# g8a9/multi-modal-emotion

Hardware: AMD Instinct MI355X
Metric: utterances/sec fwd+bwd (+clip_grad_norm_+AdamW inside the timed step), TAV (BERT+Wav2Vec2+VideoMAE) b=32, 1/2/4/8 MI355X (higher is better)
Workload: dtype bf16; 1 GPU; tav_nn.py TAV preset B (bert 12 L + wav2vec2 12 L / 768 + videomae 12 L / 768 on 16 frames + fusion 12 L), global batch 32 = 32 per GPU x 1, text 128 tok, audio 80000 samples, video 16x3x224x224 (104 fusion / 1464 encoder tokens), 547.0 GFLOP forward per utterance; global_batch=32, per_gpu_batch=32, parallelism=dp1, weights=random init (seeded), no checkpoints offline, launch=hipGraph replay

## Files before the change

### multi-modal-emotion_amd/csrc/attention.hip

```cpp
#include "common.h"
#include <type_traits>
#include "tavhip_internal.h"


namespace tav {

struct AttnP {
    const char* q; const char* k; const char* v; char* o; char* o_soft;
    const float* mask; float* lse; float* corr;
    const char* dout; char* dq; char* dk; char* dv; float* delta;
    int B, S, nh;
    long ld_q, ld_k, ld_v, ld_o, ld_do, ld_dq, ld_dk, ld_dv;
    float scale;
    int pre;
    int tiles;
};
struct AttnPL : AttnP { const int* lens; };
template <bool LEN> using AttnArg = std::conditional_t<LEN, AttnPL, AttnP>;

struct AttnTile { int x, head, b; };
TAV_DEV AttnTile attn_tile(const AttnP& p) {
    const int id = xcd_remap((int)blockIdx.x, (int)gridDim.x);
    const int hb = id / p.tiles, b = hb / p.nh;
    AttnTile w;
// ... 26 lines not shown
    static constexpr int NSD = ROWCH / 4;
    static constexpr int PITCH_N = ROWB + (ES == 2 ? 32 : 16);
    static constexpr bool DUAL = (ES == 2);
    static TAV_DEV int row_off(int row, int chunk) {
        return row * ROWB + ((chunk ^ (ES == 2 ? (((row >> 1) & 3) << 1) : (row & 15))) << 4);
    }
};

TAV_DEV uint4 frag_tr_rowimg(const char* img, int krow0, int dt, int lane) {
    using H = HD<bf16>;
    const int g = lane >> 4, i = lane & 15, q = i >> 2, p = i & 3;
    const int r0 = krow0 + 4 * g + q, r1 = r0 + 16;
    const uint2 lo = lds_read_tr16(img + H::row_off(r0, 2 * dt + (p >> 1)) + 8 * (p & 1));
    const uint2 hi = lds_read_tr16(img + H::row_off(r1, 2 * dt + (p >> 1)) + 8 * (p & 1));
    return make_uint4(lo.x, lo.y, hi.x, hi.y);
}
template <typename T> TAV_DEV float tile_elem(const char* rowimg, const char* natimg, int row, int d) {
    if constexpr (HD<T>::DUAL) return ET<T>::ld(reinterpret_cast<const T*>(rowimg + HD<T>::row_off(row, d >> 3)) + (d & 7));
    else return ET<T>::ld(reinterpret_cast<const T*>(natimg + row * HD<T>::PITCH_N) + d);
}
template <typename T> TAV_DEV uint4 tile_kfrag(const char* rowimg, const char* natimg, int krow0, int dt, int lane) {
    if constexpr (HD<T>::DUAL) return frag_tr_rowimg(rowimg, krow0, dt, lane);
    else return frag_kstrided<T>(natimg, HD<T>::PITCH_N, krow0, 16 * dt, lane);
}

template <typename T, int ROWS, int N>
TAV_DEV void tile_addr_init(unsigned (&off0)[N], unsigned (&offmax)[N], long ld_bytes, int S, int tid) {
    constexpr int ROWCH = HD<T>::ROWCH;
    static_assert(N == ROWS * ROWCH / 256, "chunks per thread");
#pragma unroll
    for (int e = 0; e < N; ++e) {
        const int idx = tid + 256 * e, row = idx / ROWCH, ch = idx - row * ROWCH;
        off0[e] = (unsigned)(row * ld_bytes + ch * 16);
        offmax[e] = (unsigned)((S - 1) * ld_bytes + ch * 16);
    }
}
template <int N>
TAV_DEV void tile_gload(uint4 (&regs)[N], const char* base, const unsigned (&off0)[N], const unsigned (&offmax)[N], unsigned tile_off) {
#pragma unroll
    for (int e = 0; e < N; ++e) {
        unsigned o = off0[e] + tile_off;
        o = o < offmax[e] ? o : offmax[e];
        typedef unsigned u32x4 __attribute__((ext_vector_type(4)));
        const u32x4 v = *reinterpret_cast<const u32x4*>(base + o);
        regs[e] = make_uint4(v.x, v.y, v.z, v.w);
    }
}

template <typename T, int ROWS>
TAV_DEV void tile_zero_pad(uint4* regs, int row0, int S, int tid) {
    constexpr int ROWCH = HD<T>::ROWCH, N = ROWS * ROWCH / 256;
#pragma unroll
    for (int e = 0; e < N; ++e) {
        const int idx = tid + 256 * e, row = idx / ROWCH;
        if (row0 + row >= S) regs[e] = make_uint4(0, 0, 0, 0);
    }
}
template <typename T, int ROWS>
TAV_DEV void tile_lstore_row(const uint4* regs, char* img, int tid) {
    constexpr int ROWCH = HD<T>::ROWCH, N = ROWS * ROWCH / 256;
#pragma unroll
    for (int e = 0; e < N; ++e) {
        const int idx = tid + 256 * e, row = idx / ROWCH, ch = idx - row * ROWCH;
        *reinterpret_cast<uint4*>(img + HD<T>::row_off(row, ch)) = regs[e];
    }
}
template <typename T, int ROWS>
TAV_DEV void tile_lstore_nat(const uint4* regs, char* img, int tid) {
    constexpr int ROWCH = HD<T>::ROWCH, N = ROWS * ROWCH / 256;
#pragma unroll
    for (int e = 0; e < N; ++e) {
        const int idx = tid + 256 * e, row = idx / ROWCH, ch = idx - row * ROWCH;
        *reinterpret_cast<uint4*>(img + row * HD<T>::PITCH_N + ch * 16) = regs[e];
    }
}

template <typename T>
TAV_DEV void row_frags_gload(uint4* f, const char* base, long ld_bytes, int r, int S, int g) {
    if (r >= S) r = S - 1;
#pragma unroll
    for (int s = 0; s < HD<T>::NSD; ++s) f[s] = *reinterpret_cast<const uint4*>(base + (long)r * ld_bytes + (4 * s + g) * 16);
}

template <int ROWS = 64> struct PairDmaT {
    static constexpr int NP = ROWS / 32;
    const char* a; const char* b;
    unsigned lda_b, ldb_b;
    unsigned offa[NP], offb[NP];
    unsigned lds_a, lds_b;
    int S, wave;
    TAV_DEV void init(const char* a_, const char* b_, long lda_bytes, long ldb_bytes, int S_, const void* lds_img_a, const void* lds_img_b, int tid) {
        a = a_; b = b_; lda_b = (unsigned)lda_bytes; ldb_b = (unsigned)ldb_bytes; S = S_;
        const int lane = tid & 63;
        wave = tid >> 6;
#pragma unroll
        for (int j = 0; j < NP; ++j) {
            const int row = wave * 8 * NP + j * 8 + (lane >> 3), slot = lane & 7;
            const int ch = slot ^ (((row >> 1) & 3) << 1);
            offa[j] = (unsigned)row * lda_b + (unsigned)(ch * 16);
            offb[j] = (unsigned)row * ldb_b + (unsigned)(ch * 16);
        }
        lds_a = __builtin_amdgcn_readfirstlane(lds_addr(lds_img_a) + wave * 8 * NP * 128);
        lds_b = __builtin_amdgcn_readfirstlane(lds_addr(lds_img_b) + wave * 8 * NP * 128);
    }
    template <bool RAGGED> TAV_DEV void issue(int t, unsigned slot_bytes) const {
        const char* ab = a + (size_t)t * (unsigned)ROWS * lda_b;
        const char* bb = b + (size_t)t * (unsigned)ROWS * ldb_b;
        unsigned oa[NP], ob[NP];
#pragma unroll
        for (int j = 0; j < NP; ++j) { oa[j] = offa[j]; ob[j] = offb[j]; }
        if constexpr (RAGGED) {
            int ln = threadIdx.x & 63;
            asm volatile("" : "+v"(ln));
#pragma unroll
            for (int j = 0; j < NP; ++j) {
                const int over = t * ROWS + wave * 8 * NP + j * 8 + (ln >> 3) - (S - 1);
                if (over > 0) { oa[j] -= (unsigned)over * lda_b; ob[j] -= (unsigned)over * ldb_b; }
            }
        }
        if constexpr (NP == 2) glds16_x4(ab, bb, oa[0], oa[1], ob[0], ob[1], lds_a + slot_bytes, lds_b + slot_bytes);
        else glds16_x2(ab, bb, oa[0], ob[0], lds_a + slot_bytes, lds_b + slot_bytes);
    }
};
using PairDma = PairDmaT<64>;

constexpr int ATT_FWD_OCC = 3;
constexpr float ATT_LAZY_THR = 12.0f;
constexpr int ATT_FWD_NQ = 2;
template <typename T, int MODE, bool PRE, bool LEN = false>
__global__ __launch_bounds__(256, ATT_FWD_OCC) void attn_fwd_kernel(const AttnArg<LEN> p) {
    constexpr int NQ = ATT_FWD_NQ;
    using H = HD<T>;
    constexpr int ES = H::ES, NSD = H::NSD, KSTEP = ET<T>::KSTEP, BKV = 64;
    constexpr int NCH = BKV * H::ROWCH / 256;
    constexpr bool DMA = ES == 2;
    constexpr int KROW_B = BKV * H::ROWB, VNAT_B = DMA ? BKV * H::ROWB : BKV * H::PITCH_N;
    constexpr int BUF_B = KROW_B + VNAT_B + 2 * BKV * 4;
    constexpr int NBUF = 2;
    extern __shared__ __attribute__((aligned(16))) char smem[];
    float* red = reinterpret_cast<float*>(smem + NBUF * BUF_B);

    const int tid = threadIdx.x, lane = tid & 63, wave = tid >> 6, g = lane >> 4, i = lane & 15;
    const AttnTile wg = attn_tile(p);
    const int head = wg.head, b = wg.b, S = p.S, L = valid_len<LEN>(p, b);
    const int q0 = wg.x * (64 * NQ) + wave * (16 * NQ);
    if constexpr (LEN) {
        if (wg.x * (64 * NQ) >= L) {
            zero_head_rows<T>(p.o, p.ld_o, b, S, head, wg.x * (64 * NQ), 64 * NQ, tid);
            if (MODE == 2) zero_head_rows<T>(p.o_soft, p.ld_o, b, S, head, wg.x * (64 * NQ), 64 * NQ, tid);
            if (tid < 64 * NQ && wg.x * (64 * NQ) + tid < S) p.lse[((long)b * p.nh + head) * S + wg.x * (64 * NQ) + tid] = 0.f;
            if (MODE == 2 && wg.x == 0 && tid < 64) p.corr[((long)b * p.nh + head) * 64 + tid] = 0.f;
            return;
        }
    }
    const long hoff = (long)head * 64 * ES;
    const char* Qb = p.q + (long)b * S * p.ld_q * ES + hoff;
    const char* Kb = p.k + (long)b * S * p.ld_k * ES + hoff;
    const char* Vb = p.v + (long)b * S * p.ld_v * ES + hoff;
    const float* maskb = p.mask ? p.mask + (long)b * S : nullptr;

    uint4 qf[NQ][NSD];
#pragma unroll
    for (int qt = 0; qt < NQ; ++qt) row_frags_gload<T>(qf[qt], Qb, p.ld_q * ES, q0 + 16 * qt + i, L, g);

    constexpr float LOG2E = 1.4426950408889634f;
    const float c2 = PRE ? 1.0f : p.scale * LOG2E;
    const uint4 ones = (ES == 2) ? make_uint4(0x3F803F80u, 0x3F803F80u, 0x3F803F80u, 0x3F803F80u)
                                 : make_uint4(0x3F800000u, 0x3F800000u, 0x3F800000u, 0x3F800000u);
    uint4 ones_v = ones;
    asm volatile("" : "+v"(ones_v.x), "+v"(ones_v.y), "+v"(ones_v.z), "+v"(ones_v.w));
    unsigned koff[NSD], vtoff[4];
    if constexpr (ES == 2) {
#pragma unroll
        for (int s = 0; s < NSD; ++s) { koff[s] = (unsigned)H::row_off(i, 4 * s + g); asm volatile("" : "+v"(koff[s])); }
#pragma unroll
        for (int dt = 0; dt < 4; ++dt) {
            vtoff[dt] = (unsigned)(H::row_off(4 * g + (i >> 2), 2 * dt + ((i & 3) >> 1)) + 8 * (i & 1));
            asm volatile("" : "+v"(vtoff[dt]));
        }
    }
    float m_run[NQ];
    f32x4 mneg[NQ];
    f32x4 lacc[NQ];
    f32x4 oacc[4][NQ];
#pragma unroll
    for (int qt = 0; qt < NQ; ++qt) {
        m_run[qt] = -1e30f;
        mneg[qt] = f32x4{0.f, 0.f, 0.f, 0.f};
        lacc[qt] = f32x4{0.f, 0.f, 0.f, 0.f};
#pragma unroll
        for (int a = 0; a < 4; ++a) oacc[a][qt] = f32x4{0.f, 0.f, 0.f, 0.f};
    }
    float corr_part = 0.f;
// ... 183 lines not shown
                f32x4 tl[2];
                tl[0] = sacc[ks * ET<T>::ACC_TILES][qt];
                tl[1] = sacc[ks * ET<T>::ACC_TILES + ET<T>::ACC_TILES - 1][qt];
                pb[qt] = acc_to_kfrag<T>(tl);
            }
#pragma unroll
            for (int qt = 0; qt < NQ; ++qt) mma16<T>(ones_v, pb[qt], lacc[qt]);
#pragma unroll
            for (int dt = 0; dt < 4; ++dt) {
                uint4 a;
                if constexpr (DMA) {
                    const char* vt = Vnat + vtoff[dt] + ks * KSTEP * H::ROWB;
                    const uint2 lo = lds_read_tr16(vt), hi = lds_read_tr16(vt + 16 * H::ROWB);
                    a = make_uint4(lo.x, lo.y, hi.x, hi.y);
                }
                else a = frag_kstrided<T>(Vnat, H::PITCH_N, ks * KSTEP, 16 * dt, lane);
#pragma unroll
                for (int qt = 0; qt < NQ; ++qt) mma16<T>(a, pb[qt], oacc[dt][qt]);
            }
        }
        if (MODE == 2) {
            const int d = tid & 63, kq = tid >> 6;
#pragma unroll 4
            for (int kk = 0; kk < 16; ++kk) {
                const int key = kq * 16 + kk;
                if constexpr (DMA) corr_part += cm[key] * ET<T>::ld(reinterpret_cast<const T*>(Vnat + H::row_off(key, d >> 3)) + (d & 7));
                else corr_part += cm[key] * ET<T>::ld(reinterpret_cast<const T*>(Vnat + key * H::PITCH_N) + d);
            }
        }
        if constexpr (NEXT != 0 && (MODE != 0 || NEXT == 2 || !DMA)) lstore(t + 1, nxt);
        if constexpr (DMA) wait_vmcnt0();
        __syncthreads();
    };
    using K0 = std::integral_constant<int, (MODE == 1) ? 1 : 0>;
    int t = 0;
    for (; t + 2 < nkt; ++t) tile_body(t, K0{}, std::integral_constant<int, 1>{});
    if (t + 1 < nkt) { tile_body(t, K0{}, std::integral_constant<int, 2>{}); ++t; }
    tile_body(t, TagYes{}, std::integral_constant<int, 0>{});

    if (MODE == 2) {
        red[wave * 64 + lane] = corr_part;
        __syncthreads();
        if (tid < 64) {
            const float c = red[tid] + red[64 + tid] + red[128 + tid] + red[192 + tid];
            red[256 + tid] = c;
            if (wg.x == 0) p.corr[((long)b * p.nh + head) * 64 + tid] = c;
        }
        __syncthreads();
    }
#pragma unroll
    for (int qt = 0; qt < NQ; ++qt) {
        const float l = lacc[qt][0];
        const int q = q0 + 16 * qt + i;
        if (q < L) {
            const float inv = 1.f / l;
            T* orow = reinterpret_cast<T*>(p.o) + ((long)b * S + q) * p.ld_o + head * 64;
            T* srow = reinterpret_cast<T*>(p.o_soft) + ((long)b * S + q) * p.ld_o + head * 64;
#pragma unroll
            for (int dt = 0; dt < 4; ++dt) {
                f32x4 v = oacc[dt][qt] * inv;
                if (MODE == 2) {
                    st4(srow + 16 * dt + 4 * g, v);
                    v += *reinterpret_cast<const f32x4*>(red + 256 + 16 * dt + 4 * g);
                }
                st4(orow + 16 * dt + 4 * g, v);
            }
            if (g == 0) p.lse[((long)b * p.nh + head) * S + q] = (m_run[qt] + log2f(l)) * 0.6931471805599453f;
        } else if (LEN && q < S) {
            T* orow = reinterpret_cast<T*>(p.o) + ((long)b * S + q) * p.ld_o + head * 64;
            T* srow = reinterpret_cast<T*>(p.o_soft) + ((long)b * S + q) * p.ld_o + head * 64;
            const f32x4 z = {0.f, 0.f, 0.f, 0.f};
#pragma unroll
            for (int dt = 0; dt < 4; ++dt) {
                if (MODE == 2) st4(srow + 16 * dt + 4 * g, z);
                st4(orow + 16 * dt + 4 * g, z);
            }
            if (g == 0) p.lse[((long)b * p.nh + head) * S + q] = 0.f;
        }
    }
}

template <typename T, int MODE, bool PRE> constexpr bool dkdv_fast32() { return sizeof(T) == 2 && MODE == 0 && PRE; }
template <typename T, int MODE, bool PRE> constexpr int dkdv_bq() { return sizeof(T) == 2 ? (dkdv_fast32<T, MODE, PRE>() ? 32 : 64) : 32; }

constexpr int ATT_DKDV_OCC = 2, ATT_DQ_OCC = 2;
template <typename T, int MODE, bool PRE, bool LEN = false>
__global__ __launch_bounds__(256, (dkdv_fast32<T, MODE, PRE>() ? 3 : ATT_DKDV_OCC)) void attn_bwd_dkdv_kernel(const AttnArg<LEN> p) {
    using H = HD<T>;
    constexpr int ES = H::ES, NSD = H::NSD, KSTEP = ET<T>::KSTEP, BQ = dkdv_bq<T, MODE, PRE>(), NQT = BQ / 16;
    constexpr int NCH = BQ * H::ROWCH / 256;
    constexpr bool DMA = ES == 2;
    constexpr int ROW_B = BQ * H::ROWB, NAT_B = H::DUAL ? 0 : BQ * H::PITCH_N;
    constexpr int BUF_B = 2 * ROW_B + 2 * NAT_B + 2 * BQ * 4;
    extern __shared__ __attribute__((aligned(16))) char smem[];
    float* red = reinterpret_cast<float*>(smem + 2 * BUF_B);

    const int tid = threadIdx.x, lane = tid & 63, wave = tid >> 6, g = lane >> 4, i = lane & 15;
    const AttnTile wg = attn_tile(p);
    const int head = wg.head, b = wg.b, S = p.S, L = valid_len<LEN>(p, b);
    const int k0 = wg.x * 128 + wave * 32;
    if constexpr (LEN) {
        if (wg.x * 128 >= L) {
            zero_head_rows<T>(p.dk, p.ld_dk, b, S, head, wg.x * 128, 128, tid);
            zero_head_rows<T>(p.dv, p.ld_dv, b, S, head, wg.x * 128, 128, tid);
            return;
        }
    }
    const long hoff = (long)head * 64 * ES;
    const char* Qb = p.q + (long)b * S * p.ld_q * ES + hoff;
    const char* Kb = p.k + (long)b * S * p.ld_k * ES + hoff;
    const char* Vb = p.v + (long)b * S * p.ld_v * ES + hoff;
    const char* dOb = p.dout + (long)b * S * p.ld_do * ES + hoff;
    const float* lseb = p.lse + ((long)b * p.nh + head) * S;
    const float* deltab = p.delta + ((long)b * p.nh + head) * S;

    uint4 kf[2][NSD], vf[2][NSD];
    float kadd[2], cmk[2];
#pragma unroll
    for (int kt = 0; kt < 2; ++kt) {
        const int key = k0 + 16 * kt + i;
        row_frags_gload<T>(kf[kt], Kb, p.ld_k * ES, key, L, g);
        row_frags_gload<T>(vf[kt], Vb, p.ld_v * ES, key, L, g);
        const bool ok = key < L;
        const float mv = (MODE != 0 && ok) ? p.mask[(long)b * S + key] : 0.f;
        kadd[kt] = ok ? (MODE == 1 ? mv * 1.4426950408889634f : 0.f) : -INFINITY;
        cmk[kt] = (MODE == 2) ? mv : 0.f;
    }
    const float c2 = PRE ? 1.0f : p.scale * 1.4426950408889634f, lse_mul = PRE ? 1.4426950408889634f : 1.0f / p.scale;
    const float dk_mul = PRE ? 0.6931471805599453f : p.scale;
    f32x4 dVt[4][2], dKt[4][2];
#pragma unroll
    for (int a = 0; a < 4; ++a)
#pragma unroll
        for (int c = 0; c < 2; ++c) { dVt[a][c] = f32x4{0.f, 0.f, 0.f, 0.f}; dKt[a][c] = f32x4{0.f, 0.f, 0.f, 0.f}; }
    float dosum_part = 0.f;

    const bool with_kadd = (MODE == 1) || (k0 + 32 > L);
    const int nqt = (L + BQ - 1) / BQ;
    uint4 rq[NCH], rdo[NCH];
    float r_lse = 0.f, r_delta = 0.f;
    unsigned q_off0[NCH], q_max[NCH], do_off0[NCH], do_max[NCH];
    if constexpr (!DMA) {
        tile_addr_init<T, BQ>(q_off0, q_max, p.ld_q * ES, L, tid);
        tile_addr_init<T, BQ>(do_off0, do_max, p.ld_do * ES, L, tid);
    }
    const unsigned qstep_b = (unsigned)(BQ * p.ld_q * ES), dostep_b = (unsigned)(BQ * p.ld_do * ES);
    PairDmaT<(ES == 2 ? BQ : 64)> qd;
    if constexpr (DMA) qd.init(Qb, dOb, p.ld_q * ES, p.ld_do * ES, L, smem, smem + ROW_B, tid);
    unsigned roff[NSD], toff[4];
    if constexpr (ES == 2) {
#pragma unroll
        for (int s = 0; s < NSD; ++s) { roff[s] = (unsigned)H::row_off(i, 4 * s + g); asm volatile("" : "+v"(roff[s])); }
#pragma unroll
        for (int dt = 0; dt < 4; ++dt) {
            toff[dt] = (unsigned)(H::row_off(4 * g + (i >> 2), 2 * dt + ((i & 3) >> 1)) + 8 * (i & 1));
            asm volatile("" : "+v"(toff[dt]));
        }
    }
    auto gload = [&](int t) {
        if constexpr (!DMA) {
            tile_gload(rq, Qb, q_off0, q_max, t * qstep_b);
            tile_gload(rdo, dOb, do_off0, do_max, t * dostep_b);
        }
        if (tid < BQ) {
            int q = t * BQ + tid;
            q = q < L ? q : L - 1;
            r_lse = lseb[q];
            r_delta = deltab[q];
        }
    };
    auto lstore = [&](int t, int buf) {
        char* base = smem + buf * BUF_B;
        if constexpr (!DMA) {
            tile_zero_pad<T, BQ>(rq, t * BQ, L, tid);
            tile_zero_pad<T, BQ>(rdo, t * BQ, L, tid);
            tile_lstore_row<T, BQ>(rq, base, tid);
            tile_lstore_row<T, BQ>(rdo, base + ROW_B, tid);
            if constexpr (!H::DUAL) {
                tile_lstore_nat<T, BQ>(rq, base + 2 * ROW_B, tid);
                tile_lstore_nat<T, BQ>(rdo, base + 2 * ROW_B + NAT_B, tid);
            }
        }
        if (tid < BQ) {
            const bool ok = t * BQ + tid < L;
            float* f = reinterpret_cast<float*>(base + 2 * ROW_B + 2 * NAT_B);
            f[tid] = ok ? -r_lse * lse_mul : -INFINITY;
            f[BQ + tid] = ok ? -r_delta : 0.f;
        }
    };
    if constexpr (DMA) { if (nqt == 1) qd.template issue<true>(0, 0u); else qd.template issue<false>(0, 0u); }
    gload(0); lstore(0, 0);
#pragma unroll
    for (int kt = 0; kt < 2; ++kt) {
#pragma unroll
        for (int s = 0; s < NSD; ++s) { settle(kf[kt][s]); settle(vf[kt][s]); }
        settle(kadd[kt]); settle(cmk[kt]);
    }
    if constexpr (DMA) wait_vmcnt0();
    __syncthreads();

    auto tile_body = [&](const int t, auto next_tag) __attribute__((always_inline)) {
        constexpr int NEXT = decltype(next_tag)::value;
        const int cur = t & 1;
        if constexpr (NEXT != 0) {
            if constexpr (DMA) qd.template issue<NEXT == 2>(t + 1, (unsigned)((cur ^ 1) * BUF_B));
            gload(t + 1);
        }
        const char* Qrow = smem + cur * BUF_B;
        const char* dOrow = Qrow + ROW_B;
        const char* Qnat = Qrow + 2 * ROW_B;
        const char* dOnat = Qnat + NAT_B;
        const float* lse_s = reinterpret_cast<const float*>(dOnat + NAT_B);
        const float* delta_s = lse_s + BQ;
        const int qbase = t * BQ;

        f32x4 sacc[NQT][2], dpacc[NQT][2];
#pragma unroll
        for (int a = 0; a < NQT; ++a) {
            const f32x4 L = *reinterpret_cast<const f32x4*>(lse_s + 16 * a + 4 * g);
            const f32x4 D = *reinterpret_cast<const f32x4*>(delta_s + 16 * a + 4 * g);
#pragma unroll
            for (int c = 0; c < 2; ++c) { sacc[a][c] = L; dpacc[a][c] = D; }
        }
        constexpr int NKS = BQ / KSTEP;
#pragma unroll
        for (int s = 0; s < NSD; ++s)
#pragma unroll
            for (int qt = 0; qt < NQT; ++qt) {
                uint4 aq, ad;
                if constexpr (ES == 2) {
                    aq = *reinterpret_cast<const uint4*>(Qrow + roff[s] + qt * 16 * H::ROWB);
                    ad = *reinterpret_cast<const uint4*>(dOrow + roff[s] + qt * 16 * H::ROWB);
                } else {
                    aq = *reinterpret_cast<const uint4*>(Qrow + H::row_off(16 * qt + i, 4 * s + g));
                    ad = *reinterpret_cast<const uint4*>(dOrow + H::row_off(16 * qt + i, 4 * s + g));
                }
                mma16<T>(aq, kf[0][s], sacc[qt][0]);
                mma16<T>(aq, kf[1][s], sacc[qt][1]);
                mma16<T>(ad, vf[0][s], dpacc[qt][0]);
                mma16<T>(ad, vf[1][s], dpacc[qt][1]);
            }
#pragma unroll
        for (int qt = 0; qt < NQT; ++qt) {
            if (with_kadd) {
#pragma unroll
                for (int kt = 0; kt < 2; ++kt) {
                    float ka = kadd[kt];
                    if constexpr (MODE != 1) { int ky = k0 + 16 * kt + i; asm volatile("" : "+v"(ky)); ka = ky < L ? 0.f : -INFINITY; }
#pragma unroll
                    for (int r = 0; r < 4; ++r) sacc[qt][kt][r] = fast_exp2(PRE ? sacc[qt][kt][r] + ka : __builtin_fmaf(sacc[qt][kt][r], c2, ka));
                }
            } else {
#pragma unroll
                for (int kt = 0; kt < 2; ++kt)
#pragma unroll
                    for (int r = 0; r < 4; ++r) sacc[qt][kt][r] = fast_exp2(PRE ? sacc[qt][kt][r] : sacc[qt][kt][r] * c2);
            }
#pragma unroll
            for (int kt = 0; kt < 2; ++kt)
#pragma unroll
                for (int r = 0; r < 4; ++r) dpacc[qt][kt][r] *= sacc[qt][kt][r];
        }
#pragma unroll
        for (int ks = 0; ks < NKS; ++ks) {
            uint4 pb[2], dsb[2];
#pragma unroll
            for (int kt = 0; kt < 2; ++kt) {
                f32x4 tl[2];
                tl[0] = sacc[ks * ET<T>::ACC_TILES][kt]; tl[1] = sacc[ks * ET<T>::ACC_TILES + ET<T>::ACC_TILES - 1][kt];
                pb[kt] = acc_to_kfrag<T>(tl);
                tl[0] = dpacc[ks * ET<T>::ACC_TILES][kt]; tl[1] = dpacc[ks * ET<T>::ACC_TILES + ET<T>::ACC_TILES - 1][kt];
                dsb[kt] = acc_to_kfrag<T>(tl);
            }
#pragma unroll
            for (int dt = 0; dt < 4; ++dt) {
                uint4 a1, a2;
                if constexpr (ES == 2) {
                    const char* t1 = dOrow + toff[dt] + ks * KSTEP * H::ROWB;
                    const char* t2 = Qrow + toff[dt] + ks * KSTEP * H::ROWB;
                    const uint2 lo1 = lds_read_tr16(t1), hi1 = lds_read_tr16(t1 + 16 * H::ROWB);
                    const uint2 lo2 = lds_read_tr16(t2), hi2 = lds_read_tr16(t2 + 16 * H::ROWB);
                    a1 = make_uint4(lo1.x, lo1.y, hi1.x, hi1.y);
                    a2 = make_uint4(lo2.x, lo2.y, hi2.x, hi2.y);
                } else {
                    a1 = tile_kfrag<T>(dOrow, dOnat, ks * KSTEP, dt, lane);
                    a2 = tile_kfrag<T>(Qrow, Qnat, ks * KSTEP, dt, lane);
                }
                mma16<T>(a1, pb[0], dVt[dt][0]);
                mma16<T>(a1, pb[1], dVt[dt][1]);
                mma16<T>(a2, dsb[0], dKt[dt][0]);
                mma16<T>(a2, dsb[1], dKt[dt][1]);
            }
        }
        if (MODE == 2) {
            const int d = tid & 63, rq8 = tid >> 6;
#pragma unroll
            for (int rr = 0; rr < BQ / 4; ++rr) {
                const int row = rq8 * (BQ / 4) + rr;
                const float v = tile_elem<T>(dOrow, dOnat, row, d);
                dosum_part += (!DMA || qbase + row < L) ? v : 0.f;
            }
        }
        if constexpr (NEXT != 0) lstore(t + 1, cur ^ 1);
        if constexpr (DMA) wait_vmcnt0();
        __syncthreads();
    };
    int t = 0;
    for (; t + 2 < nqt; ++t) tile_body(t, std::integral_constant<int, 1>{});
    if (t + 1 < nqt) { tile_body(t, std::integral_constant<int, 2>{}); ++t; }
    tile_body(t, std::integral_constant<int, 0>{});

    if (MODE == 2) {
        red[wave * 64 + lane] = dosum_part;
        __syncthreads();
        if (tid < 64) red[256 + tid] = red[tid] + red[64 + tid] + red[128 + tid] + red[192 + tid];
        __syncthreads();
    }
#pragma unroll
    for (int kt = 0; kt < 2; ++kt) {
        const int key = k0 + 16 * kt + i;
        if (key < L) {
            T* dkrow = reinterpret_cast<T*>(p.dk) + ((long)b * S + key) * p.ld_dk + head * 64;
            T* dvrow = reinterpret_cast<T*>(p.dv) + ((long)b * S + key) * p.ld_dv + head * 64;
#pragma unroll
            for (int dt = 0; dt < 4; ++dt) {
                f32x4 dvv = dVt[dt][kt];
                if (MODE == 2) dvv += *reinterpret_cast<const f32x4*>(red + 256 + 16 * dt + 4 * g) * cmk[kt];
                st4(dvrow + 16 * dt + 4 * g, dvv);
                st4(dkrow + 16 * dt + 4 * g, dKt[dt][kt] * dk_mul);
            }
        } else if (LEN && key < S) {
            T* dkrow = reinterpret_cast<T*>(p.dk) + ((long)b * S + key) * p.ld_dk + head * 64;
            T* dvrow = reinterpret_cast<T*>(p.dv) + ((long)b * S + key) * p.ld_dv + head * 64;
            const f32x4 z = {0.f, 0.f, 0.f, 0.f};
#pragma unroll
            for (int dt = 0; dt < 4; ++dt) { st4(dvrow + 16 * dt + 4 * g, z); st4(dkrow + 16 * dt + 4 * g, z); }
        }
    }
}

template <typename T, int MODE, bool PRE, bool LEN = false>
__global__ __launch_bounds__(256, (sizeof(T) == 2 ? ATT_DQ_OCC : 1)) void attn_bwd_dq_kernel(const AttnArg<LEN> p) {
    using H = HD<T>;
    constexpr int ES = H::ES, NSD = H::NSD, KSTEP = ET<T>::KSTEP, BKV = 64;
    constexpr int NCH = BKV * H::ROWCH / 256;
    constexpr bool DMA = ES == 2;
    constexpr int ROW_B = BKV * H::ROWB, NAT_B = H::DUAL ? 0 : BKV * H::PITCH_N;
    constexpr int BUF_B = 2 * ROW_B + NAT_B + BKV * 4;
    extern __shared__ __attribute__((aligned(16))) char smem[];

    const int tid = threadIdx.x, lane = tid & 63, wave = tid >> 6, g = lane >> 4, i = lane & 15;
    const AttnTile wg = attn_tile(p);
    const int head = wg.head, b = wg.b, S = p.S, L = valid_len<LEN>(p, b);
    const int q0 = wg.x * 128 + wave * 32;
    if constexpr (LEN) {
        if (wg.x * 128 >= L) {
            zero_head_rows<T>(p.dq, p.ld_dq, b, S, head, wg.x * 128, 128, tid);
            return;
        }
    }
    const long hoff = (long)head * 64 * ES;
    const char* Qb = p.q + (long)b * S * p.ld_q * ES + hoff;
    const char* Kb = p.k + (long)b * S * p.ld_k * ES + hoff;
    const char* Vb = p.v + (long)b * S * p.ld_v * ES + hoff;
    const char* dOb = p.dout + (long)b * S * p.ld_do * ES + hoff;
    const float* maskb = p.mask ? p.mask + (long)b * S : nullptr;

    uint4 qf[2][NSD], dof[2][NSD];
    float lse_q[2], delta_q[2];
#pragma unroll
    for (int qt = 0; qt < 2; ++qt) {
        int q = q0 + 16 * qt + i;
        row_frags_gload<T>(qf[qt], Qb, p.ld_q * ES, q, L, g);
        row_frags_gload<T>(dof[qt], dOb, p.ld_do * ES, q, L, g);
        if (q >= L) q = L - 1;
        lse_q[qt] = -p.lse[((long)b * p.nh + head) * S + q] * (PRE ? 1.4426950408889634f : 1.0f / p.scale);
        const char* Ob = (MODE == 2 ? p.o_soft : p.o) + ((long)b * S * p.ld_o + (long)head * 64) * ES;
        uint4 of[NSD];
        row_frags_gload<T>(of, Ob, p.ld_o * ES, q, L, g);
        float part = 0.f;
#pragma unroll
        for (int s = 0; s < NSD; ++s) {
            const uint32_t ow[4] = {of[s].x, of[s].y, of[s].z, of[s].w}, dw[4] = {dof[qt][s].x, dof[qt][s].y, dof[qt][s].z, dof[qt][s].w};
#pragma unroll
            for (int e = 0; e < 4; ++e) {
                if constexpr (ES == 2) {
                    part = __builtin_fmaf(bf16_bits_to_f32(ow[e] & 0xffffu), bf16_bits_to_f32(dw[e] & 0xffffu), part);
                    part = __builtin_fmaf(__uint_as_float(ow[e] & 0xffff0000u), __uint_as_float(dw[e] & 0xffff0000u), part);
                } else part = __builtin_fmaf(__uint_as_float(ow[e]), __uint_as_float(dw[e]), part);
            }
        }
        part = sum_over_row_groups(part);
        delta_q[qt] = -part;
// ... 82 lines not shown
#pragma unroll
        for (int s = 0; s < NSD; ++s)
#pragma unroll
            for (int kt = 0; kt < 4; ++kt) {
                uint4 ak, av;
                if constexpr (ES == 2) {
                    ak = *reinterpret_cast<const uint4*>(Krow + koff[s] + kt * 16 * H::ROWB);
                    av = *reinterpret_cast<const uint4*>(Vrow + koff[s] + kt * 16 * H::ROWB);
                } else {
                    ak = *reinterpret_cast<const uint4*>(Krow + H::row_off(16 * kt + i, 4 * s + g));
                    av = *reinterpret_cast<const uint4*>(Vrow + H::row_off(16 * kt + i, 4 * s + g));
                }
                mma16<T>(ak, qf[0][s], sacc[kt][0]);
                mma16<T>(ak, qf[1][s], sacc[kt][1]);
                mma16<T>(av, dof[0][s], dpacc[kt][0]);
                mma16<T>(av, dof[1][s], dpacc[kt][1]);
            }
        if constexpr (KADD) {
#pragma unroll
            for (int kt = 0; kt < 4; ++kt) {
                const f32x4 ka = *reinterpret_cast<const f32x4*>(kadd + 16 * kt + 4 * g);
#pragma unroll
                for (int qt = 0; qt < 2; ++qt)
#pragma unroll
                    for (int r = 0; r < 4; ++r) sacc[kt][qt][r] = fast_exp2(PRE ? sacc[kt][qt][r] + ka[r] : __builtin_fmaf(sacc[kt][qt][r], c2, ka[r])) * dpacc[kt][qt][r];
            }
        } else {
#pragma unroll
            for (int kt = 0; kt < 4; ++kt)
#pragma unroll
                for (int qt = 0; qt < 2; ++qt)
#pragma unroll
                    for (int r = 0; r < 4; ++r) sacc[kt][qt][r] = fast_exp2(PRE ? sacc[kt][qt][r] : sacc[kt][qt][r] * c2) * dpacc[kt][qt][r];
        }
#pragma unroll
        for (int ks = 0; ks < NKS; ++ks) {
            uint4 dsb[2];
#pragma unroll
            for (int qt = 0; qt < 2; ++qt) {
                f32x4 tl[2];
                tl[0] = sacc[ks * ET<T>::ACC_TILES][qt]; tl[1] = sacc[ks * ET<T>::ACC_TILES + ET<T>::ACC_TILES - 1][qt];
                dsb[qt] = acc_to_kfrag<T>(tl);
            }
#pragma unroll
            for (int dt = 0; dt < 4; ++dt) {
                uint4 a;
                if constexpr (ES == 2) {
                    const char* kt_ = Krow + ktoff[dt] + ks * KSTEP * H::ROWB;
                    const uint2 lo = lds_read_tr16(kt_), hi = lds_read_tr16(kt_ + 16 * H::ROWB);
                    a = make_uint4(lo.x, lo.y, hi.x, hi.y);
                } else a = tile_kfrag<T>(Krow, Knat, ks * KSTEP, dt, lane);
                mma16<T>(a, dsb[0], dQt[dt][0]);
                mma16<T>(a, dsb[1], dQt[dt][1]);
            }
        }
        if constexpr (NEXT != 0) lstore(t + 1, cur ^ 1);
        if constexpr (DMA) wait_vmcnt0();
        __syncthreads();
    };
    using K0 = std::integral_constant<int, (MODE == 1) ? 1 : 0>;
    int t = 0;
    for (; t + 2 < nkt; ++t) tile_body(t, K0{}, std::integral_constant<int, 1>{});
    if (t + 1 < nkt) { tile_body(t, K0{}, std::integral_constant<int, 2>{}); ++t; }
    tile_body(t, std::integral_constant<int, 1>{}, std::integral_constant<int, 0>{});
#pragma unroll
    for (int qt = 0; qt < 2; ++qt) {
        const int q = q0 + 16 * qt + i;
        if (q < L) {
            T* dqrow = reinterpret_cast<T*>(p.dq) + ((long)b * S + q) * p.ld_dq + head * 64;
#pragma unroll
            for (int dt = 0; dt < 4; ++dt) st4(dqrow + 16 * dt + 4 * g, dQt[dt][qt] * p.scale);
        } else if (LEN && q < S) {
            T* dqrow = reinterpret_cast<T*>(p.dq) + ((long)b * S + q) * p.ld_dq + head * 64;
#pragma unroll
            for (int dt = 0; dt < 4; ++dt) st4(dqrow + 16 * dt + 4 * g, f32x4{0.f, 0.f, 0.f, 0.f});
        }
    }
}

template <typename T> constexpr size_t fwd_lds() {
    return 2 * (64 * HD<T>::ROWB + 64 * HD<T>::PITCH_N + 2 * 64 * 4) + (256 + 64) * 4;
}
template <typename T, int MODE, bool PRE> constexpr size_t dkdv_lds() {
    constexpr int BQ = dkdv_bq<T, MODE, PRE>();
    return 2 * (2 * BQ * HD<T>::ROWB + (HD<T>::DUAL ? 0 : 2 * BQ * HD<T>::PITCH_N) + 2 * BQ * 4) + (256 + 64) * 4;
}
template <typename T> constexpr size_t dq_lds() { return 2 * (2 * 64 * HD<T>::ROWB + (HD<T>::DUAL ? 0 : 64 * HD<T>::PITCH_N) + 64 * 4); }

template <typename T>
__global__ __launch_bounds__(256) void attn_probs_kernel(const AttnP p, float* __restrict__ probs, const float* __restrict__ hs, int hs_bstride, int mode) {
    constexpr int ES = ET<T>::ES;
    constexpr float L2E = 1.4426950408889634f;
    const int lane = threadIdx.x & 63, wave = threadIdx.x >> 6;
    const long row = (long)blockIdx.x * 4 + wave;
    if (row >= (long)p.B * p.nh * p.S) return;
    const int i = (int)(row % p.S), head = (int)((row / p.S) % p.nh), b = (int)(row / ((long)p.S * p.nh));
    const T* qr = reinterpret_cast<const T*>(p.q + ((long)(b * p.S + i) * p.ld_q + head * 64) * ES);
    f32x4 qv[16];
#pragma unroll
    for (int t = 0; t < 16; ++t) qv[t] = ld4(qr + 4 * t);
    const float c = p.pre ? 1.f : p.scale * L2E;
    const float l2 = p.lse[((long)b * p.nh + head) * p.S + i] * L2E;
    const float f = hs ? hs[(long)b * hs_bstride + head] : 1.f;
    for (int j = lane; j < p.S; j += 64) {
        const T* kr = reinterpret_cast<const T*>(p.k + ((long)(b * p.S + j) * p.ld_k + head * 64) * ES);
        float dot = 0.f;
#pragma unroll
        for (int t = 0; t < 16; ++t) { const f32x4 kv = ld4(kr + 4 * t); dot += qv[t][0] * kv[0] + qv[t][1] * kv[1] + qv[t][2] * kv[2] + qv[t][3] * kv[3]; }
        float s2 = dot * c;
        if (mode == 1) s2 += p.mask[(long)b * p.S + j] * L2E;
        float pr = exp2f(s2 - l2) * f;
        if (mode == 2) pr += p.mask[(long)b * p.S + j];
        probs[row * p.S + j] = pr;
    }
}
template <typename T>
__global__ void head_scale_kernel(const T* __restrict__ a, const T* __restrict__ bsrc, T* __restrict__ out, const float* __restrict__ hs, int hs_bstride,
                                  float c0, long n4, int S, int nh, long lda, long ldb, long ldo) {
    const long i4 = (long)blockIdx.x * blockDim.x + threadIdx.x;
    if (i4 >= n4) return;
    const long row = i4 / (nh * 16);
    const int col4 = (int)(i4 - row * (nh * 16)), head = col4 >> 4;
    const float f = c0 + (hs ? hs[(row / S) * hs_bstride + head] : 0.f);
    f32x4 v = ld4(bsrc + row * ldb + 4 * col4) * f;
    if (a) v += ld4(a + row * lda + 4 * col4);
    st4(out + row * ldo + 4 * col4, v);
}

static int check(const tav_attn_args* a, bool bwd) {
    if (!a || !a->q || !a->k || !a->v || !a->o || !a->lse) return TAV_ERR_NULL;
    if (a->B <= 0 || a->S <= 0 || a->nheads <= 0) return TAV_ERR_SHAPE;
    if (((a->S + 63) / 64) * a->nheads * a->B >= (1ll << 31)) return TAV_ERR_SHAPE;
    if (a->dtype != TAV_BF16 && a->dtype != TAV_F32) return TAV_ERR_DTYPE;
    if (a->mask_mode < 0 || a->mask_mode > 2) return TAV_ERR_SHAPE;
    if (a->mask_mode != 0 && !a->key_mask) return TAV_ERR_NULL;
    if (a->mask_mode == 2 && (!a->corr || !a->o_soft)) return TAV_ERR_NULL;
    const int pk = a->dtype == TAV_BF16 ? 8 : 4;
    if (a->ld_q % pk || a->ld_k % pk || a->ld_v % pk || a->ld_o % 4) return TAV_ERR_ALIGN;
    if (a->ld_q < a->nheads * 64 || a->ld_k < a->nheads * 64 || a->ld_v < a->nheads * 64 || a->ld_o < a->nheads * 64) return TAV_ERR_SHAPE;
    {
        const int64_t es = a->dtype == TAV_BF16 ? 2 : 4;
        int64_t ld = a->ld_q > a->ld_k ? a->ld_q : a->ld_k;
        ld = ld > a->ld_v ? ld : a->ld_v;
        if (bwd && a->ld_do > ld) ld = a->ld_do;
        if ((a->S + 64) * ld * es >= (1ll << 32)) return TAV_ERR_SHAPE;
    }
    if (bwd) {
        if (!a->dout || !a->dq || !a->dk || !a->dv || !a->delta) return TAV_ERR_NULL;
        if (a->ld_do % pk || a->ld_dq % 4 || a->ld_dk % 4 || a->ld_dv % 4) return TAV_ERR_ALIGN;
    }
    return 0;
}
static AttnP pack(const tav_attn_args* a) {
    AttnP p;
    p.q = (const char*)a->q; p.k = (const char*)a->k; p.v = (const char*)a->v; p.o = (char*)a->o; p.o_soft = (char*)a->o_soft;
    p.mask = a->key_mask; p.lse = a->lse; p.corr = a->corr;
    p.dout = (const char*)a->dout; p.dq = (char*)a->dq; p.dk = (char*)a->dk; p.dv = (char*)a->dv; p.delta = a->delta;
    p.B = (int)a->B; p.S = (int)a->S; p.nh = (int)a->nheads;
    p.ld_q = a->ld_q; p.ld_k = a->ld_k; p.ld_v = a->ld_v; p.ld_o = a->ld_o; p.ld_do = a->ld_do;
    p.ld_dq = a->ld_dq; p.ld_dk = a->ld_dk; p.ld_dv = a->ld_dv;
    p.scale = a->scale;
    p.pre = a->q_prescaled != 0;
    p.tiles = 1;
    return p;
}

template <typename T, int MODE, bool PRE, bool LEN> static int launch_fwd(const AttnArg<LEN>& p, hipStream_t st) {
// ... 102 lines not shown
```

Before: 428.0 utterances/s.

## Stage 64-row Q/dO tiles in dK/dV fast path, compute in two 32-row passes

For the bf16 unmasked pre-scaled dK/dV backward kernel, Q and dO are now staged through LDS in 64-row tiles while compute still runs over 32-row sub-passes. This halves the number of DMA issue, wait and barrier rounds per key block. The kernel also specialises the loop on whether the key-mask add is needed, recomputes the second DMA row offset to save registers, and loads lse and delta with one split thread range. In exchange it uses more LDS per block, which may reduce occupancy at the declared 3 blocks per CU.

```diff
diff --git a/multi-modal-emotion_amd/csrc/attention.hip b/multi-modal-emotion_amd/csrc/attention.hip
--- a/multi-modal-emotion_amd/csrc/attention.hip
+++ b/multi-modal-emotion_amd/csrc/attention.hip
@@ -132,11 +132,12 @@
     for (int s = 0; s < HD<T>::NSD; ++s) f[s] = *reinterpret_cast<const uint4*>(base + (long)r * ld_bytes + (4 * s + g) * 16);
 }
 
-template <int ROWS = 64> struct PairDmaT {
+template <int ROWS = 64, bool LEAN = false> struct PairDmaT {
     static constexpr int NP = ROWS / 32;
+    static constexpr int NK = LEAN ? 1 : NP;
     const char* a; const char* b;
     unsigned lda_b, ldb_b;
-    unsigned offa[NP], offb[NP];
+    unsigned offa[NK], offb[NK];
     unsigned lds_a, lds_b;
     int S, wave;
     TAV_DEV void init(const char* a_, const char* b_, long lda_bytes, long ldb_bytes, int S_, const void* lds_img_a, const void* lds_img_b, int tid) {
@@ -144,7 +145,7 @@
         const int lane = tid & 63;
         wave = tid >> 6;
 #pragma unroll
-        for (int j = 0; j < NP; ++j) {
+        for (int j = 0; j < NK; ++j) {
             const int row = wave * 8 * NP + j * 8 + (lane >> 3), slot = lane & 7;
             const int ch = slot ^ (((row >> 1) & 3) << 1);
             offa[j] = (unsigned)row * lda_b + (unsigned)(ch * 16);
@@ -158,7 +159,12 @@
         const char* bb = b + (size_t)t * (unsigned)ROWS * ldb_b;
         unsigned oa[NP], ob[NP];
 #pragma unroll
-        for (int j = 0; j < NP; ++j) { oa[j] = offa[j]; ob[j] = offb[j]; }
+        for (int j = 0; j < NK; ++j) { oa[j] = offa[j]; ob[j] = offb[j]; }
+        if constexpr (NK < NP) {
+            unsigned a0 = offa[0], b0 = offb[0];
+            asm volatile("" : "+v"(a0), "+v"(b0));
+            oa[1] = a0 + 8u * lda_b; ob[1] = b0 + 8u * ldb_b;
+        }
         if constexpr (RAGGED) {
             int ln = threadIdx.x & 63;
             asm volatile("" : "+v"(ln));
@@ -508,16 +514,20 @@
 
 template <typename T, int MODE, bool PRE> constexpr bool dkdv_fast32() { return sizeof(T) == 2 && MODE == 0 && PRE; }
 template <typename T, int MODE, bool PRE> constexpr int dkdv_bq() { return sizeof(T) == 2 ? (dkdv_fast32<T, MODE, PRE>() ? 32 : 64) : 32; }
+template <typename T, int MODE, bool PRE> constexpr int dkdv_stage() { return dkdv_fast32<T, MODE, PRE>() ? 64 : dkdv_bq<T, MODE, PRE>(); }
 
 constexpr int ATT_DKDV_OCC = 2, ATT_DQ_OCC = 2;
 template <typename T, int MODE, bool PRE, bool LEN = false>
 __global__ __launch_bounds__(256, (dkdv_fast32<T, MODE, PRE>() ? 3 : ATT_DKDV_OCC)) void attn_bwd_dkdv_kernel(const AttnArg<LEN> p) {
     using H = HD<T>;
     constexpr int ES = H::ES, NSD = H::NSD, KSTEP = ET<T>::KSTEP, BQ = dkdv_bq<T, MODE, PRE>(), NQT = BQ / 16;
-    constexpr int NCH = BQ * H::ROWCH / 256;
+    constexpr int BS = dkdv_stage<T, MODE, PRE>(), NPASS = BS / BQ;
+    constexpr int NCH = BS * H::ROWCH / 256;
     constexpr bool DMA = ES == 2;
-    constexpr int ROW_B = BQ * H::ROWB, NAT_B = H::DUAL ? 0 : BQ * H::PITCH_N;
-    constexpr int BUF_B = 2 * ROW_B + 2 * NAT_B + 2 * BQ * 4;
+    constexpr int ROW_B = BS * H::ROWB, NAT_B = H::DUAL ? 0 : BS * H::PITCH_N;
+    constexpr int BUF_B = 2 * ROW_B + 2 * NAT_B + 2 * BS * 4;
+    constexpr bool FAST = dkdv_fast32<T, MODE, PRE>();
+    static_assert(NPASS == 1 || H::DUAL, "a second pass addresses the row image only");
     extern __shared__ __attribute__((aligned(16))) char smem[];
     float* red = reinterpret_cast<float*>(smem + 2 * BUF_B);
 
@@ -561,17 +571,17 @@
         for (int c = 0; c < 2; ++c) { dVt[a][c] = f32x4{0.f, 0.f, 0.f, 0.f}; dKt[a][c] = f32x4{0.f, 0.f, 0.f, 0.f}; }
     float dosum_part = 0.f;
 
-    const bool with_kadd = (MODE == 1) || (k0 + 32 > L);
-    const int nqt = (L + BQ - 1) / BQ;
+    const bool with_kadd = (MODE == 1) || (dkdv_fast32<T, MODE, PRE>() ? wg.x * 128 + __builtin_amdgcn_readfirstlane(wave) * 32 + 32 > L : k0 + 32 > L);
+    const int nqt = (L + BS - 1) / BS;
     uint4 rq[NCH], rdo[NCH];
     float r_lse = 0.f, r_delta = 0.f;
     unsigned q_off0[NCH], q_max[NCH], do_off0[NCH], do_max[NCH];
     if constexpr (!DMA) {
-        tile_addr_init<T, BQ>(q_off0, q_max, p.ld_q * ES, L, tid);
-        tile_addr_init<T, BQ>(do_off0, do_max, p.ld_do * ES, L, tid);
-    }
-    const unsigned qstep_b = (unsigned)(BQ * p.ld_q * ES), dostep_b = (unsigned)(BQ * p.ld_do * ES);
-    PairDmaT<(ES == 2 ? BQ : 64)> qd;
+        tile_addr_init<T, BS>(q_off0, q_max, p.ld_q * ES, L, tid);
+        tile_addr_init<T, BS>(do_off0, do_max, p.ld_do * ES, L, tid);
+    }
+    const unsigned qstep_b = (unsigned)(BS * p.ld_q * ES), dostep_b = (unsigned)(BS * p.ld_do * ES);
+    PairDmaT<(ES == 2 ? BS : 64), dkdv_fast32<T, MODE, PRE>()> qd;
     if constexpr (DMA) qd.init(Qb, dOb, p.ld_q * ES, p.ld_do * ES, L, smem, smem + ROW_B, tid);
     unsigned roff[NSD], toff[4];
     if constexpr (ES == 2) {
@@ -588,8 +598,17 @@
             tile_gload(rq, Qb, q_off0, q_max, t * qstep_b);
             tile_gload(rdo, dOb, do_off0, do_max, t * dostep_b);
         }
-        if (tid < BQ) {
-            int q = t * BQ + tid;
+        if constexpr (FAST) {
+            int tl = threadIdx.x;
+            asm volatile("" : "+v"(tl));
+            if (tl < 2 * BS) {
+                const float* src = __builtin_amdgcn_readfirstlane(tl) < BS ? lseb : deltab;
+                int q = t * BS + (tl & (BS - 1));
+                q = q < L ? q : L - 1;
+                r_lse = src[q];
+            }
+        } else if (tid < BS) {
+            int q = t * BS + tid;
             q = q < L ? q : L - 1;
             r_lse = lseb[q];
             r_delta = deltab[q];
@@ -598,20 +617,28 @@
     auto lstore = [&](int t, int buf) {
         char* base = smem + buf * BUF_B;
         if constexpr (!DMA) {
-            tile_zero_pad<T, BQ>(rq, t * BQ, L, tid);
-            tile_zero_pad<T, BQ>(rdo, t * BQ, L, tid);
-            tile_lstore_row<T, BQ>(rq, base, tid);
-            tile_lstore_row<T, BQ>(rdo, base + ROW_B, tid);
+            tile_zero_pad<T, BS>(rq, t * BS, L, tid);
+            tile_zero_pad<T, BS>(rdo, t * BS, L, tid);
+            tile_lstore_row<T, BS>(rq, base, tid);
+            tile_lstore_row<T, BS>(rdo, base + ROW_B, tid);
             if constexpr (!H::DUAL) {
-                tile_lstore_nat<T, BQ>(rq, base + 2 * ROW_B, tid);
-                tile_lstore_nat<T, BQ>(rdo, base + 2 * ROW_B + NAT_B, tid);
-            }
-        }
-        if (tid < BQ) {
-            const bool ok = t * BQ + tid < L;
+                tile_lstore_nat<T, BS>(rq, base + 2 * ROW_B, tid);
+                tile_lstore_nat<T, BS>(rdo, base + 2 * ROW_B + NAT_B, tid);
+            }
+        }
+        if constexpr (FAST) {
+            int tl = threadIdx.x;
+            asm volatile("" : "+v"(tl));
+            if (tl < 2 * BS) {
+                const bool ok = t * BS + (tl & (BS - 1)) < L;
+                float* f = reinterpret_cast<float*>(base + 2 * ROW_B + 2 * NAT_B);
+                f[tl] = tl < BS ? (ok ? -r_lse * lse_mul : -INFINITY) : (ok ? -r_lse : 0.f);
+            }
+        } else if (tid < BS) {
+            const bool ok = t * BS + tid < L;
             float* f = reinterpret_cast<float*>(base + 2 * ROW_B + 2 * NAT_B);
             f[tid] = ok ? -r_lse * lse_mul : -INFINITY;
-            f[BQ + tid] = ok ? -r_delta : 0.f;
+            f[BS + tid] = ok ? -r_delta : 0.f;
         }
     };
     if constexpr (DMA) { if (nqt == 1) qd.template issue<true>(0, 0u); else qd.template issue<false>(0, 0u); }
@@ -625,20 +652,16 @@
     if constexpr (DMA) wait_vmcnt0();
     __syncthreads();
 
-    auto tile_body = [&](const int t, auto next_tag) __attribute__((always_inline)) {
-        constexpr int NEXT = decltype(next_tag)::value;
-        const int cur = t & 1;
-        if constexpr (NEXT != 0) {
-            if constexpr (DMA) qd.template issue<NEXT == 2>(t + 1, (unsigned)((cur ^ 1) * BUF_B));
-            gload(t + 1);
-        }
-        const char* Qrow = smem + cur * BUF_B;
+    auto pass_body = [&](const int t, const int cur, auto h_tag, auto kadd_tag) __attribute__((always_inline)) {
+        constexpr int HP = decltype(h_tag)::value;
+        constexpr int KADD = decltype(kadd_tag)::value;
+        const char* Qrow = smem + cur * BUF_B + HP * BQ * H::ROWB;
         const char* dOrow = Qrow + ROW_B;
-        const char* Qnat = Qrow + 2 * ROW_B;
+        const char* Qnat = smem + cur * BUF_B + 2 * ROW_B;
         const char* dOnat = Qnat + NAT_B;
-        const float* lse_s = reinterpret_cast<const float*>(dOnat + NAT_B);
-        const float* delta_s = lse_s + BQ;
-        const int qbase = t * BQ;
+        const float* lse_s = reinterpret_cast<const float*>(dOnat + NAT_B) + HP * BQ;
+        const float* delta_s = lse_s + BS;
+        const int qbase = t * BS + HP * BQ;
 
         f32x4 sacc[NQT][2], dpacc[NQT][2];
 #pragma unroll
@@ -668,7 +691,7 @@
             }
 #pragma unroll
         for (int qt = 0; qt < NQT; ++qt) {
-            if (with_kadd) {
+            if (KADD == 1 || (KADD == 2 && with_kadd)) {
 #pragma unroll
                 for (int kt = 0; kt < 2; ++kt) {
                     float ka = kadd[kt];
@@ -727,14 +750,32 @@
                 dosum_part += (!DMA || qbase + row < L) ? v : 0.f;
             }
         }
+    };
+    auto tile_body = [&](const int t, auto next_tag, auto kadd_tag) __attribute__((always_inline)) {
+        constexpr int NEXT = decltype(next_tag)::value;
+        const int cur = t & 1;
+        if constexpr (NEXT != 0) {
+            if constexpr (DMA) qd.template issue<NEXT == 2>(t + 1, (unsigned)((cur ^ 1) * BUF_B));
+            gload(t + 1);
+        }
+        pass_body(t, cur, std::integral_constant<int, 0>{}, kadd_tag);
+        if constexpr (NPASS == 2) {
+            if (NEXT != 0 || t * BS + BQ < L) pass_body(t, cur, std::integral_constant<int, 1>{}, kadd_tag);
+        }
         if constexpr (NEXT != 0) lstore(t + 1, cur ^ 1);
         if constexpr (DMA) wait_vmcnt0();
+        if constexpr (FAST) settle(r_lse);
         __syncthreads();
     };
-    int t = 0;
-    for (; t + 2 < nqt; ++t) tile_body(t, std::integral_constant<int, 1>{});
-    if (t + 1 < nqt) { tile_body(t, std::integral_constant<int, 2>{}); ++t; }
-    tile_body(t, std::integral_constant<int, 0>{});
+    auto stage_loop = [&](auto kadd_tag) __attribute__((always_inline)) {
+        int t = 0;
+        for (; t + 2 < nqt; ++t) tile_body(t, std::integral_constant<int, 1>{}, kadd_tag);
+        if (t + 1 < nqt) { tile_body(t, std::integral_constant<int, 2>{}, kadd_tag); ++t; }
+        tile_body(t, std::integral_constant<int, 0>{}, kadd_tag);
+    };
+    if constexpr (!dkdv_fast32<T, MODE, PRE>()) stage_loop(std::integral_constant<int, 2>{});
+    else if (with_kadd) stage_loop(std::integral_constant<int, 1>{});
+    else stage_loop(std::integral_constant<int, 0>{});
 
     if (MODE == 2) {
         red[wave * 64 + lane] = dosum_part;
@@ -983,7 +1024,7 @@
     return 2 * (64 * HD<T>::ROWB + 64 * HD<T>::PITCH_N + 2 * 64 * 4) + (256 + 64) * 4;
 }
 template <typename T, int MODE, bool PRE> constexpr size_t dkdv_lds() {
-    constexpr int BQ = dkdv_bq<T, MODE, PRE>();
+    constexpr int BQ = dkdv_stage<T, MODE, PRE>();
     return 2 * (2 * BQ * HD<T>::ROWB + (HD<T>::DUAL ? 0 : 2 * BQ * HD<T>::PITCH_N) + 2 * BQ * 4) + (256 + 64) * 4;
 }
 template <typename T> constexpr size_t dq_lds() { return 2 * (2 * 64 * HD<T>::ROWB + (HD<T>::DUAL ? 0 : 64 * HD<T>::PITCH_N) + 64 * 4); }
```

Result: no change. 429.4 utterances/s (median of 6 runs) (+0.3%).
